# avik-pal/LocalRegNeuralDE.jl

Measured on AMD Instinct MI355X. Metric: NFE/s (vector-field evals/s inside the adaptive Tsit5 NeuralODE forward, MNIST-ODE B=512/GPU), higher is better.
Workload: dtype f32; 1 GPU; MNIST-ODE MLP field TDChain(Dense(785=>100,tanh),Dense(101=>784)), B=512/GPU, Tsit5 adaptive abstol=reltol=1.4e-08, tspan=(0,1), regularize=unbiased/error_estimate, forward pass (solve + local reg step); global_batch=512, parallelism=batch-shard x1

## Files before the change

localregneuralde.jl_amd/csrc/lrnde_qtile.hpp:

```cpp

constexpr int QNB = 4;
constexpr int QNW = 7;
constexpr int QNT = QNW * 64;
constexpr int QB1 = 7;
constexpr int QSEG = 28;
constexpr int QB2 = 4;
constexpr int QRGC = 4;

struct SmemQ {
  f32x4* xl;
  f32x4* hl;
  f32x4* pl;
  float* bias;
  double* red;
  Bcast* bc;
};

__device__ __forceinline__ int q_nseg1(const ModelDev& m) { return (m.KQ1p + QSEG - 1) / QSEG; }
__host__ __device__ __forceinline__ int q_w2_groups(int KQ1p) { return 2 * ((KQ1p + QSEG - 1) / QSEG); }

__device__ __forceinline__ float q_segment_sum(const float* plf, int ne, int e, int nseg) {
  float vals[QNW];
#pragma unroll
  for (int sgi = 0; sgi < QNW; ++sgi) vals[sgi] = plf[(size_t)(sgi < nseg ? sgi : nseg - 1) * ne + e];
// ... 206 lines not shown
#pragma unroll
    for (int r = 0; r < 4; ++r) {
      float sum = (float)Tsit5::BT[0] * k1[r] + (float)Tsit5::BT[1] * k2[r];
      sum = sum + (float)Tsit5::BT[2] * k3[r];
      sum = sum + (float)Tsit5::BT[3] * k4[r];
      sum = sum + (float)Tsit5::BT[4] * k5[r];
      sum = sum + (float)Tsit5::BT[5] * k6[r];
      sum = sum + (float)Tsit5::BT[6] * kv[r];
      const float utilde = dt * sum;
      const float sc = abstol + fmaxf_(__builtin_fabsf(up[r]), __builtin_fabsf(pb[0][r])) * reltol;
      const float rr = utilde / sc;
      const float sq = rr * rr;
      *aerr += (double)sq;
      if (want_stiff) {
        const float d1 = pb[0][r] - pb[1][r];
        const float d2 = kv[r] - k6[r];
        const float q1 = d1 * d1, q2 = d2 * d2;
        *aden += (double)q1; *anum += (double)q2;
      }
    }
  }
};

template <int S> struct EpiStageQL {
  static constexpr int NPRE = S;
  TileIOQ io;
  int off_up, off_k[6], off_out, off_x;
  float dt;
  f32x4* xl;
  f32x4* kl; int KL;
  const f32x4* klu; const f32x4* klk;
  int store_k;
  template <class G> __device__ __forceinline__ void pre(G, int rb, bool, f32x4 (&pb)[NPRE]) const {
    const int li = rb + (threadIdx.x & 63);
    pb[0] = klu[li];
    if (S > 1) pb[S > 1 ? 1 : 0] = klk[li];
#pragma unroll
    for (int j = 2; j < S; ++j) pb[j] = kl[(size_t)(j + 2) * KL + li];
  }
  template <class G> __device__ __forceinline__ void post(G, int rb, bool own, const f32x4& kv, f32x4 (&pb)[NPRE]) const {
    const int lane = threadIdx.x & 63, sidx = lane & 3, q = lane >> 2;
    constexpr int off = (S - 1) * S / 2;
    const int vo = q_voff(io, rb, own);
    qstore(io, store_k ? vo : 0x7ffffff0, off_out, kv);
    if (own) kl[(size_t)(S + 2) * KL + rb + lane] = kv;
    f32x4 x;
#pragma unroll
    for (int r = 0; r < 4; ++r) {
      float o[S];
#pragma unroll
      for (int j = 0; j < S - 1; ++j) o[j] = pb[1 + j][r];
      o[S - 1] = kv[r];
      float sum = (float)Tsit5::A[off] * o[0] + (float)Tsit5::A[off + 1] * o[1];
#pragma unroll
      for (int j = 2; j < S; ++j) sum = sum + (float)Tsit5::A[off + j] * o[j];
      x[r] = pb[0][r] + dt * sum;
    }
    if (off_x >= 0) qstore(io, vo, off_x, x);
    if (own) xl[(rb / 4 + q) * 4 + sidx] = x;
  }
};

struct EpiFinalQL {
  static constexpr int NPRE = 9;
  TileIOQ io;
  int off_up, off_u, off_k[6], off_g6, off_out;
  float dt, abstol, reltol;
  int want_stiff, nvalid, D;
  double *aerr, *anum, *aden;
  const f32x4* xl; const f32x4* kl; int KL;
  const f32x4* klu; const f32x4* klk;
  __amdgpu_buffer_rsrc_t rsD; int nstB; bool rec;
  template <class G> __device__ __forceinline__ void pre(G, int rb, bool own, f32x4 (&pb)[NPRE]) const {
    const int li = rb + (threadIdx.x & 63);
    pb[0] = klu[li];
    pb[1] = xl[li];
    pb[2] = klk[li];
#pragma unroll
    for (int j = 1; j < 6; ++j) pb[2 + j] = kl[(size_t)(3 + j) * KL + li];
    if (want_stiff) pb[8] = qload(io, q_voff(io, rb, own), off_g6);
  }
  template <class G> __device__ __forceinline__ void post(G, int rb, bool own, const f32x4& kv, f32x4 (&pb)[NPRE]) const {
    const int lane = threadIdx.x & 63, sidx = lane & 3;
    const int vo = q_voff(io, rb, own);
    qstore(io, vo, off_out, kv);
    if (rec) {
      const int vd = vo;
      f32x4 P2, P3, P4;
#pragma unroll
      for (int r = 0; r < 4; ++r) {
        const float kk[6] = {pb[3][r], pb[4][r], pb[5][r], pb[6][r], pb[7][r], kv[r]};
        float P[3];
        tsit5_rec_poly(pb[2][r], kk, P);
        P2[r] = P[0]; P3[r] = P[1]; P4[r] = P[2];
      }
      __builtin_amdgcn_raw_buffer_store_b128(__builtin_bit_cast(u32x4, pb[0]), rsD, vd, 0, 0);
      __builtin_amdgcn_raw_buffer_store_b128(__builtin_bit_cast(u32x4, pb[2]), rsD, vd + nstB, 0, 0);
      __builtin_amdgcn_raw_buffer_store_b128(__builtin_bit_cast(u32x4, P2), rsD, vd + 2 * nstB, 0, 0);
      __builtin_amdgcn_raw_buffer_store_b128(__builtin_bit_cast(u32x4, P3), rsD, vd + 3 * nstB, 0, 0);
      __builtin_amdgcn_raw_buffer_store_b128(__builtin_bit_cast(u32x4, P4), rsD, vd + 4 * nstB, 0, 0);
    }
    if (sidx >= nvalid || !own) return;
#pragma unroll
    for (int r = 0; r < 4; ++r) {
      float sum = (float)Tsit5::BT[0] * pb[2][r] + (float)Tsit5::BT[1] * pb[3][r];
      sum = sum + (float)Tsit5::BT[2] * pb[4][r];
      sum = sum + (float)Tsit5::BT[3] * pb[5][r];
      sum = sum + (float)Tsit5::BT[4] * pb[6][r];
      sum = sum + (float)Tsit5::BT[5] * pb[7][r];
      sum = sum + (float)Tsit5::BT[6] * kv[r];
      const float utilde = dt * sum;
      const float sc = abstol + fmaxf_(__builtin_fabsf(pb[0][r]), __builtin_fabsf(pb[1][r])) * reltol;
      const float rr = utilde / sc;
      const float sq = rr * rr;
      *aerr += (double)sq;
      if (want_stiff) {
        const float d1 = pb[1][r] - pb[8][r];
        const float d2 = kv[r] - pb[7][r];
        const float q1 = d1 * d1, q2 = d2 * d2;
        *aden += (double)q1; *anum += (double)q2;
      }
    }
  }
};


constexpr int QSQ = 4;
constexpr int QSB1 = QSEG / QSQ;
constexpr int QSB2 = 7;
constexpr int QSB = QSB1 + QSB2;
#ifndef LRNDE_QRING
#define LRNDE_QRING 3
#endif
constexpr int QRING = LRNDE_QRING;
constexpr int QAHEAD = QRING - 1;
constexpr int VRING = 3;
#ifndef LRNDE_QPARK
#define LRNDE_QPARK 0x1040u
#endif
constexpr unsigned QPARK = LRNDE_QPARK;
__host__ __device__ constexpr int q_popcount(unsigned v) { int n = 0; for (; v; v &= v - 1) ++n; return n; }
__host__ __device__ constexpr int q_park_nb(unsigned mask) { return q_popcount(mask & ((1u << QSB) - 1)); }
__host__ __device__ constexpr int q_park_index(unsigned mask, int B) { return q_popcount(mask & ((1u << B) - 1)); }
__host__ __device__ constexpr int q_park_block(unsigned mask, int P) {
  for (int B = 0; B < QSB; ++B) if ((mask >> B) & 1u) { if (P == 0) return B; --P; }
  return -1;
}
constexpr int QPARK_FRAG = QSQ * 2;
__host__ __device__ constexpr size_t q_park_bytes(unsigned mask) { return (size_t)QNW * q_park_nb(mask) * QPARK_FRAG * 1024; }
static_assert((QPARK >> QSB) == 0, "LRNDE_QPARK is a mask over the QSB stream blocks of an f-eval");
static_assert(smem_bytes_q(7 * QSEG, QSEG, 2, 13) + q_park_bytes(QPARK) <= 160 * 1024,
              "forward layout + park region exceed the 160 KiB of LDS of a CU: park fewer blocks");

template <int I> struct IC { static constexpr int value = I; };
template <int I0, int I1, class F> __device__ __forceinline__ void static_for(F&& f) {
  if constexpr (I0 < I1) { f(IC<I0>{}); static_for<I0 + 1, I1>(f); }
}

struct StreamQ {
  __amdgpu_buffer_rsrc_t rs1, rs2;
  int v1[2], v2[2];
  int s1[2], s2[2];
  int kq2_real;
  f32x4 ring[QRING][QSQ][2];
  const f32x4* park;
};

__device__ __forceinline__ void q_barrier() {
  asm volatile("s_waitcnt lgkmcnt(0)\n\ts_barrier" ::: "memory");
}

template <int B, int SLOT>
__device__ __forceinline__ void q_stream_load(StreamQ& st) {
  if constexpr (B < QSB1) {
#pragma unroll
    for (int j = 0; j < QSQ; ++j) {
      st.ring[SLOT][j][0] = wload(st.rs1, st.v1[0], st.s1[0] + (B * QSQ + j) * 1024);
      st.ring[SLOT][j][1] = wload(st.rs1, st.v1[1], st.s1[1] + (B * QSQ + j) * 1024);
    }
  } else {
#pragma unroll
    for (int j = 0; j < QSQ; ++j) {
      constexpr int kq = (B - QSB1) * QSQ;
      const bool real = (kq + j) < st.kq2_real;
      st.ring[SLOT][j][0] = wload(st.rs2, real ? st.v2[0] : 0x7ffffff0, st.s2[0] + (kq + j) * 1024);
      st.ring[SLOT][j][1] = wload(st.rs2, real ? st.v2[1] : 0x7ffffff0, st.s2[1] + (kq + j) * 1024);
    }
  }
  __builtin_amdgcn_sched_barrier(0);
}

template <int B, int SLOT, int J, int KT = 4, unsigned PARK = 0>
__device__ __forceinline__ void q_stream_load_quad(StreamQ& st) {
#ifdef LRNDE_QABL_NOLOAD
  st.ring[SLOT][J][0] = f32x4{0.f, 0.f, 0.f, 0.f}; st.ring[SLOT][J][1] = f32x4{0.f, 0.f, 0.f, 0.f};
  asm volatile("" : "+v"(st.ring[SLOT][J][0]), "+v"(st.ring[SLOT][J][1]));
  return;
#endif
  if constexpr (((PARK >> B) & 1u) != 0) {
    if constexpr (B < QSB - 1 || J < KT) {
      constexpr int f = (q_park_index(PARK, B) * QSQ + J) * 2;
      st.ring[SLOT][J][0] = st.park[f * 64];
      st.ring[SLOT][J][1] = st.park[(f + 1) * 64];
    }
  } else if constexpr (B < QSB1) {
    st.ring[SLOT][J][0] = wload(st.rs1, st.v1[0], st.s1[0] + (B * QSQ + J) * 1024);
    st.ring[SLOT][J][1] = wload(st.rs1, st.v1[1], st.s1[1] + (B * QSQ + J) * 1024);
  } else if constexpr (B < QSB - 1 || J < KT) {
    constexpr int kq = (B - QSB1) * QSQ;
    const bool real = (kq + J) < st.kq2_real;
    st.ring[SLOT][J][0] = wload(st.rs2, real ? st.v2[0] : 0x7ffffff0, st.s2[0] + (kq + J) * 1024);
    st.ring[SLOT][J][1] = wload(st.rs2, real ? st.v2[1] : 0x7ffffff0, st.s2[1] + (kq + J) * 1024);
  }
}

__device__ __forceinline__ void stream_init_q(const ModelDev& m, StreamQ& st) {
  const int lane = threadIdx.x & 63;
  const int wave = __builtin_amdgcn_readfirstlane(threadIdx.x >> 6);
  const int voff = lane * 16;
  st.rs1 = __builtin_amdgcn_make_buffer_rsrc((void*)m.W1q, 0, m.RG1 * m.KQ1p * 1024, 0x00020000);
  st.rs2 = __builtin_amdgcn_make_buffer_rsrc((void*)m.W2q, 0, q_w2_groups(m.KQ1p) * m.KQ2p * 1024, 0x00020000);
  const bool has1 = wave < q_nseg1(m);
#pragma unroll
  for (int c = 0; c < 2; ++c) {
#ifdef LRNDE_X_FULLROWS
    st.v1[c] = (has1 && c < m.RG1) ? voff : 0x7ffffff0;
#else
    st.v1[c] = (has1 && c < m.RG1 && c * 64 + lane < m.H) ? voff : 0x7ffffff0;
#endif
    st.s1[c] = (c * m.KQ1p + (has1 ? wave * QSEG : 0)) * 1024;
    const int rb = wave * (QSEG * 4) + c * 64;
    st.v2[c] = (has1 && (c == 0 || lane < QSEG * 4 - 64) && rb + lane < m.D) ? voff : 0x7ffffff0;
    st.s2[c] = (has1 ? 2 * wave + c : 0) * m.KQ2p * 1024;
  }
  st.kq2_real = (m.H + 3) / 4;
  static_for<0, QAHEAD>([&](auto Bc) { constexpr int B = decltype(Bc)::value; q_stream_load<B, B>(st); });
}

#ifndef LRNDE_QBURST
#define LRNDE_QLOAD_QUAD(BB, SS, JJ) q_stream_load_quad<BB, SS, JJ, KT, PARK>(st)
#define LRNDE_QPIN() __builtin_amdgcn_sched_barrier(0)
#else
#define LRNDE_QLOAD_QUAD(BB, SS, JJ) do {} while (0)
#define LRNDE_QPIN() do {} while (0)
#endif
#ifdef LRNDE_QABL_NOMFMA
__device__ __forceinline__ f32x4 qmfma(float a, float b, f32x4 c) { asm volatile("" : "+v"(c) : "v"(a), "v"(b)); return c; }
#else
__device__ __forceinline__ f32x4 qmfma(float a, float b, f32x4 c) { return __builtin_amdgcn_mfma_f32_4x4x1f32(a, b, c, 0, 0, 0); }
#endif
template <class Epi, int SLOT0, int KT = 4, unsigned PARK = 0>
__device__ __forceinline__ void feval_qs(const ModelDev& m, const SmemQ& sm, StreamQ& st, float ts, const Epi& epi,
                                         const Epi1Q* ep1 = nullptr) {
  const int lane = threadIdx.x & 63;
  const int wave = __builtin_amdgcn_readfirstlane(threadIdx.x >> 6);
  const int sidx = lane & 3, q = lane >> 2;
  const f32x4 zero4 = {0.f, 0.f, 0.f, 0.f};
  const int h64 = m.RG1 * 64, d64 = m.RG2 * 64;
  const float* w2t = sm.bias + 2 * h64; const float* b2 = w2t + d64;
  const int nseg1 = q_nseg1(m);
  f32x4 acc0 = zero4, acc1 = zero4;
  STAMP(1); STAMPW(0);
  {
    const f32x4* xp = sm.xl + (size_t)((wave < nseg1 ? wave : 0) * QSEG) * 4 + sidx;
    f32x4 bq[2][QSQ];
#pragma unroll
    for (int j = 0; j < QSQ; ++j) bq[0][j] = xp[j * 4];
    static_for<0, QSB1>([&](auto Bc) {
      constexpr int B = decltype(Bc)::value;
      constexpr int SL = (SLOT0 + B) % QRING, NSL = (SLOT0 + B + QAHEAD) % QRING;
#ifdef LRNDE_QBURST
      q_stream_load<(B + QAHEAD) % QSB, NSL>(st);
#endif
      if constexpr (B + 1 < QSB1) {
#pragma unroll
        for (int j = 0; j < QSQ; ++j) bq[(B + 1) & 1][j] = xp[((B + 1) * QSQ + j) * 4];
      }
      const f32x4 (&b_)[QSQ] = bq[B & 1];
      static_for<0, QSQ>([&](auto Jc) {
        constexpr int j = decltype(Jc)::value;
        LRNDE_QLOAD_QUAD((B + QAHEAD) % QSB, NSL, j);
        acc0 = qmfma(st.ring[SL][j][0].x, b_[j].x, acc0);
        acc1 = qmfma(st.ring[SL][j][1].x, b_[j].x, acc1);
        acc0 = qmfma(st.ring[SL][j][0].y, b_[j].y, acc0);
        acc1 = qmfma(st.ring[SL][j][1].y, b_[j].y, acc1);
        acc0 = qmfma(st.ring[SL][j][0].z, b_[j].z, acc0);
        acc1 = qmfma(st.ring[SL][j][1].z, b_[j].z, acc1);
        acc0 = qmfma(st.ring[SL][j][0].w, b_[j].w, acc0);
        acc1 = qmfma(st.ring[SL][j][1].w, b_[j].w, acc1);
        LRNDE_QPIN();
      });
      __builtin_amdgcn_sched_barrier(0);
    });
    if (wave < nseg1) {
      f32x4* pp = sm.pl + ((size_t)wave * m.RG1) * 64 + lane;
      pp[0] = acc0;
      if (m.RG1 > 1) pp[64] = acc1;
    }
  }
  STAMP(2); STAMPW(1);
  q_barrier();
  STAMP(3);
  if (ep1) q_epilogue1(m, sm, *ep1, ts);
  else q_epilogue1(m, sm, q_epi1_make(m, sm), ts);
  STAMPW(2);
  q_barrier();
  STAMP(4); STAMPW(3);
  {
    const f32x4* hp = sm.hl + sidx;
    acc0 = zero4; acc1 = zero4;
    const int g0 = wave * (QSEG * 4), g1 = g0 + 64;
    const bool own0 = g0 + q * 4 < m.D, own1 = q < (QSEG * 4 - 64) / 4 && g1 + q * 4 < m.D;
    f32x4 pb0[Epi::NPRE], pb1[Epi::NPRE];
    f32x4 bq[2][QSQ];
#pragma unroll
    for (int j = 0; j < QSQ; ++j) bq[0][j] = hp[j * 4];
    static_for<0, QSB2>([&](auto Bc) {
      constexpr int B = decltype(Bc)::value;
      constexpr int SL = (SLOT0 + QSB1 + B) % QRING, NSL = (SLOT0 + QSB1 + B + QAHEAD) % QRING;
#ifdef LRNDE_QBURST
      q_stream_load<(QSB1 + B + QAHEAD) % QSB, NSL>(st);
#endif
      if constexpr (B == QSB2 - 3) {
        if (g0 < m.D) epi.pre(IC<0>{}, g0, own0, pb0);
        if (g1 < m.D) epi.pre(IC<1>{}, g1, own1, pb1);
        __builtin_amdgcn_sched_barrier(0);
      }
      if constexpr (B + 1 < QSB2) {
#pragma unroll
        for (int j = 0; j < QSQ; ++j) bq[(B + 1) & 1][j] = hp[((B + 1) * QSQ + j) * 4];
      }
      const f32x4 (&b_)[QSQ] = bq[B & 1];
      static_for<0, QSQ>([&](auto Jc) {
        constexpr int j = decltype(Jc)::value;
        LRNDE_QLOAD_QUAD((QSB1 + B + QAHEAD) % QSB, NSL, j);
        if constexpr (B < QSB2 - 1 || j < KT) {
          acc0 = qmfma(st.ring[SL][j][0].x, b_[j].x, acc0);
          acc1 = qmfma(st.ring[SL][j][1].x, b_[j].x, acc1);
          acc0 = qmfma(st.ring[SL][j][0].y, b_[j].y, acc0);
          acc1 = qmfma(st.ring[SL][j][1].y, b_[j].y, acc1);
          acc0 = qmfma(st.ring[SL][j][0].z, b_[j].z, acc0);
          acc1 = qmfma(st.ring[SL][j][1].z, b_[j].z, acc1);
          acc0 = qmfma(st.ring[SL][j][0].w, b_[j].w, acc0);
          acc1 = qmfma(st.ring[SL][j][1].w, b_[j].w, acc1);
        }
        LRNDE_QPIN();
      });
      __builtin_amdgcn_sched_barrier(0);
    });
    auto finish = [&](int rb, bool own, const f32x4& tot) {
      const int row0 = own ? rb + q * 4 : 0;
      const f32x4 wt = *reinterpret_cast<const f32x4*>(w2t + row0);
      const f32x4 bb = *reinterpret_cast<const f32x4*>(b2 + row0);
      f32x4 kv;
#pragma unroll
      for (int r = 0; r < 4; ++r) {
        const float pre = m.td ? fma_(wt[r], ts, tot[r]) : tot[r];
        kv[r] = pre + bb[r];
      }
      return kv;
    };
    if (g0 < m.D) epi.post(IC<0>{}, g0, own0, finish(g0, own0, acc0), pb0);
    if (g1 < m.D) epi.post(IC<1>{}, g1, own1, finish(g1, own1, acc1), pb1);
  }
  STAMP(5); STAMPW(4);
  __builtin_amdgcn_fence(__ATOMIC_ACQ_REL, "wavefront");
  STAMP(6);
}

template <class F>
__device__ __forceinline__ void q_tile_foreach(const ModelDev& m, int b0, int nvalid, int KQ1, F&& fn) {
  for (int i = threadIdx.x; i < KQ1 * 4; i += QNT) {
    const int sidx = i & 3, kq = i >> 2;
    fn(kq, sidx, sidx < nvalid, (size_t)(b0 + sidx) * m.D + kq * 4);
  }
}

__device__ __forceinline__ f32x4 ld4(const float* p) { return *reinterpret_cast<const f32x4*>(p); }
__device__ __forceinline__ void st4(float* p, const f32x4& v) { *reinterpret_cast<f32x4*>(p) = v; }

__device__ __forceinline__ void block_sum3_q(double* red, double& a, double& b, double& c, bool three = true) {
  const int lane = threadIdx.x & 63;
  const int wave = __builtin_amdgcn_readfirstlane(threadIdx.x >> 6);
  a = wave_sum_dpp(a);
  if (three) { b = wave_sum_dpp(b); c = wave_sum_dpp(c); }
  if (lane == 0) { red[wave * 3 + 0] = a; red[wave * 3 + 1] = b; red[wave * 3 + 2] = c; }
  __syncthreads();
  if (threadIdx.x == 0) {
    double sa = 0.0, sb = 0.0, sc = 0.0;
    for (int w = 0; w < QNW; ++w) { sa += red[w * 3]; sb += red[w * 3 + 1]; sc += red[w * 3 + 2]; }
    a = sa; b = sb; c = sc;
  }
}

__device__ __forceinline__ void q_feval_store(const ModelDev& m, const SmemQ& sm, StreamQ& fc, float ts,
                                              float* kout, int b0, int nvalid) {
  EpiStoreKQ e;
  e.m = &m; e.kout = kout; e.b0 = b0; e.nvalid = nvalid;
  feval_qs<EpiStoreKQ, 0>(m, sm, fc, ts, e);
  __syncthreads();
}

__global__ __launch_bounds__(QNT) void k_rhs_q(StepArgs a, const float* u, float t, float* du) {
  STAMP(0);
  const SmemQ s = carve_q(a.m);
  smem_init_q(a.m, s);
  StreamQ fc;
  stream_init_q(a.m, fc);
  const int b0 = blockIdx.x * QNB, nvalid = min(QNB, a.B - b0);
  const int KQ1 = a.m.D / 4;
  __syncthreads();
  q_tile_foreach(a.m, b0, nvalid, KQ1, [&](int kq, int sidx, bool valid, size_t g) {
    const f32x4 z = {0.f, 0.f, 0.f, 0.f};
    s.xl[kq * 4 + sidx] = valid ? ld4(u + g) : z;
  });
  __syncthreads();
  q_feval_store(a.m, s, fc, t, du, b0, nvalid);
}

__global__ __launch_bounds__(QNT) void k_init1_q(StepArgs a) {
  const SmemQ s = carve_q(a.m);
  smem_init_q(a.m, s);
  StreamQ fc;
  stream_init_q(a.m, fc);
  const int b0 = blockIdx.x * QNB, nvalid = min(QNB, a.B - b0);
  const int KQ1 = a.m.D / 4;
  int cur0; float tinit;
  if (a.init_fresh) {
    cur0 = 0; tinit = a.t0;
    if (blockIdx.x == 0 && threadIdx.x == 0) solve_init_body(a.ctrl, a.t0, a.init_nsaved, a.init_si);
  } else {
    const Ctrl c = a.ctrl[0];
    cur0 = c.cur; tinit = c.t;
  }
  const float* u0 = a.init_u0 ? a.init_u0 : ubuf_at(a, cur0);
  float* ucopy = a.init_u0 ? ubuf_at(a, cur0) : nullptr;
  float* f0 = kfsal_at(a, cur0);
  __syncthreads();
  q_tile_foreach(a.m, b0, nvalid, KQ1, [&](int kq, int sidx, bool valid, size_t g) {
    const f32x4 z = {0.f, 0.f, 0.f, 0.f};
    const f32x4 v = valid ? ld4(u0 + g) : z;
    s.xl[kq * 4 + sidx] = v;
    if (valid && ucopy) st4(ucopy + g, v);
  });
  __syncthreads();
  q_feval_store(a.m, s, fc, tinit, f0, b0, nvalid);
  double a0 = 0.0, a1 = 0.0, a2 = 0.0;
  q_tile_foreach(a.m, b0, nvalid, KQ1, [&](int, int, bool valid, size_t g) {
    if (!valid) return;
    const f32x4 u = ld4(u0 + g), f = ld4(f0 + g);
#pragma unroll
    for (int h = 0; h < 4; ++h) {
      const float sk = a.abstol + __builtin_fabsf(u[h]) * a.reltol;
      const float r0 = u[h] / sk, r1 = f[h] / sk;
      const float q0 = r0 * r0, q1 = r1 * r1;
      a0 += (double)q0; a1 += (double)q1;
    }
  });
  block_sum3_q(s.red, a0, a1, a2);
  publish_partial(a, 2, a0, a1, 0.0);
}

__global__ __launch_bounds__(QNT) void k_init2_q(StepArgs a) {
  const SmemQ s = carve_q(a.m);
  smem_init_q(a.m, s);
  StreamQ fc;
  stream_init_q(a.m, fc);
  const int b0 = blockIdx.x * QNB, nvalid = min(QNB, a.B - b0);
  const int KQ1 = a.m.D / 4;
  const Ctrl c = a.ctrl[0];
  if (threadIdx.x < 64) {
    double s1[3];
    reduce_partials(a.pinit_recv, a.nwg_global, s1);
    if (threadIdx.x == 0) s.bc->dt0 = init_dt0(s1, a.n_global, a.t1 - a.t0);
  }
  __syncthreads();
  const float dt0 = s.bc->dt0;
  const float* u0 = ubuf_at(a, c.cur);
  const float* f0 = kfsal_at(a, c.cur);
  float* f1 = a.ks[0];
  q_tile_foreach(a.m, b0, nvalid, KQ1, [&](int kq, int sidx, bool valid, size_t g) {
    f32x4 x = {0.f, 0.f, 0.f, 0.f};
    if (valid) {
      const f32x4 u = ld4(u0 + g), f = ld4(f0 + g);
#pragma unroll
      for (int h = 0; h < 4; ++h) x[h] = u[h] + dt0 * f[h];
    }
    s.xl[kq * 4 + sidx] = x;
  });
  __syncthreads();
  q_feval_store(a.m, s, fc, c.t + dt0, f1, b0, nvalid);
  double a0 = 0.0, a1 = 0.0, a2 = 0.0;
  q_tile_foreach(a.m, b0, nvalid, KQ1, [&](int, int, bool valid, size_t g) {
    if (!valid) return;
    const f32x4 u = ld4(u0 + g), f = ld4(f0 + g), ff = ld4(f1 + g);
#pragma unroll
    for (int h = 0; h < 4; ++h) {
      const float sk = a.abstol + __builtin_fabsf(u[h]) * a.reltol;
      const float r2 = (ff[h] - f[h]) / sk;
      const float q2 = r2 * r2;
      a0 += (double)q2;
    }
  });
  block_sum3_q(s.red, a0, a1, a2);
  publish_partial(a, 3, a0, 0.0, 0.0);
}

struct QRowOff { int v1, s1, v2, s2; };
__device__ __forceinline__ QRowOff q_row_off(const ModelDev& m, int wave, int lane, int c) {
  const int voff = lane * 16;
  const bool has1 = wave < q_nseg1(m);
  QRowOff r;
#ifdef LRNDE_X_FULLROWS
  r.v1 = (has1 && c < m.RG1) ? voff : 0x7ffffff0;
#else
  r.v1 = (has1 && c < m.RG1 && c * 64 + lane < m.H) ? voff : 0x7ffffff0;
#endif
  r.s1 = (c * m.KQ1p + (has1 ? wave * QSEG : 0)) * 1024;
  const int rb = wave * (QSEG * 4) + c * 64;
  r.v2 = (has1 && (c == 0 || lane < QSEG * 4 - 64) && rb + lane < m.D) ? voff : 0x7ffffff0;
  r.s2 = (has1 ? 2 * wave + c : 0) * m.KQ2p * 1024;
  return r;
}

template <int B>
__device__ __forceinline__ f32x4 q_park_load0(const StreamQ& st, const QRowOff& ra, const QRowOff& rb, int e, bool on) {
  const int J = e >> 1;
  const bool c1 = (e & 1) != 0;
  if constexpr (B < QSB1) {
    return wload(st.rs1, on ? (c1 ? rb.v1 : ra.v1) : 0x7ffffff0, (c1 ? rb.s1 : ra.s1) + (B * QSQ + J) * 1024);
  } else {
    const int kq = (B - QSB1) * QSQ + J;
    return wload(st.rs2, on && kq < st.kq2_real ? (c1 ? rb.v2 : ra.v2) : 0x7ffffff0, (c1 ? rb.s2 : ra.s2) + kq * 1024);
  }
}
template <unsigned PARK, int KT, int P>
__device__ __forceinline__ void q_park_fill_block(StreamQ& st, const QRowOff& ra, const QRowOff& rb, int fw, f32x4* own, f32x4* w0) {
  if constexpr (P < q_park_nb(PARK)) {
    constexpr int B = q_park_block(PARK, P), FREE = QRING - 1;
    const int e2 = QNW - 1 + fw - 2 * (P % 3);
    const bool on2 = e2 >= QNW - 1 && e2 < QPARK_FRAG;
    q_stream_load_quad<B, FREE, 0, KT, 0>(st);
    q_stream_load_quad<B, FREE, 1, KT, 0>(st);
    q_stream_load_quad<B, FREE, 2, KT, 0>(st);
    q_stream_load_quad<B, FREE, 3, KT, 0>(st);
    const f32x4 va = q_park_load0<B>(st, ra, rb, fw, true), vb = q_park_load0<B>(st, ra, rb, on2 ? e2 : 0, on2);
    __builtin_amdgcn_sched_barrier(0);
#pragma unroll
    for (int J = 0; J < QSQ; ++J) {
      if (B < QSB - 1 || J < KT) {
        own[((P * QSQ + J) * 2) * 64] = st.ring[FREE][J][0];
        own[((P * QSQ + J) * 2 + 1) * 64] = st.ring[FREE][J][1];
      }
    }
    w0[(P * QPARK_FRAG + fw) * 64] = va;
    if (on2) w0[(P * QPARK_FRAG + e2) * 64] = vb;
    __builtin_amdgcn_sched_barrier(0);
    q_park_fill_block<PARK, KT, P + 1>(st, ra, rb, fw, own, w0);
  }
}
template <unsigned PARK, int KT>
__device__ __forceinline__ void q_park_fill(const ModelDev& m, StreamQ& st, f32x4* park) {
  static_assert(QSQ == 4, "q_park_fill_block issues the four quads of a block by name");
  constexpr int NF = q_park_nb(PARK) * QPARK_FRAG;
  const int lane = threadIdx.x & 63;
  const int fw = __builtin_amdgcn_readfirstlane(threadIdx.x >> 6) - 1;
  const QRowOff ra = q_row_off(m, 0, lane, 0), rb = q_row_off(m, 0, lane, 1);
  q_park_fill_block<PARK, KT, 0>(st, ra, rb, fw, park + (size_t)(fw + 1) * (NF * 64) + lane, park + lane);
}

template <bool SPEC, int KT> __global__ __launch_bounds__(QNT) void k_step_q(StepArgs a, int j) {
  STAMP(9);
  const SmemQ s = carve_q(a.m);
  StreamQ fc;
  stream_init_q(a.m, fc);
  const int b0 = blockIdx.x * QNB, nvalid = min(QNB, a.B - b0);
  const int KQ1 = a.m.D / 4;
  STAMP(10);
  const TileIOQ io = make_tile_io_q(a, b0, nvalid);
  const int qlane = (threadIdx.x & 63) >> 2;
  const int g0 = __builtin_amdgcn_readfirstlane(threadIdx.x >> 6) * (QSEG * 4), g1 = g0 + 64;
  const bool own0 = g0 + qlane * 4 < a.m.D, own1 = qlane < (QSEG * 4 - 64) / 4 && g1 + qlane * 4 < a.m.D;
  const int vo0 = q_voff(io, g0, own0), vo1 = q_voff(io, g1, own1);
  RegOpsQ R;
#ifndef LRNDE_NO_PRELOAD
  f32x4 cu[2][2], ck[2][2];
  auto preload = [&]() {
#pragma unroll
    for (int p = 0; p < 2; ++p) {
      cu[p][0] = qload(io, vo0, arr_off(a, p)); cu[p][1] = qload(io, vo1, arr_off(a, p));
      ck[p][0] = qload(io, vo0, arr_off(a, 2 + p)); ck[p][1] = qload(io, vo1, arr_off(a, 2 + p));
    }
  };
#else
  auto preload = [&]() {};
#endif
  constexpr bool REGS = q_regops(KT);
  f32x4* kl = REGS ? nullptr : q_extra_smem(s);
  const int KL = a.m.KQ1p * 4;
  constexpr bool PARKED = REGS && QPARK != 0;
  if constexpr (PARKED) {
    constexpr int NF = q_park_nb(QPARK) * QPARK_FRAG;
    fc.park = q_extra_smem(s) + (size_t)__builtin_amdgcn_readfirstlane(threadIdx.x >> 6) * (NF * 64) + (threadIdx.x & 63);
  }
  if (threadIdx.x < 64) {
    if constexpr (REGS) preload();
    step_prologue(a, j, s.bc);
  } else {
    smem_init_q<true>(a.m, s);
    if constexpr (REGS) {
      preload();
      if constexpr (PARKED) q_park_fill<QPARK, KT>(a.m, fc, q_extra_smem(s));
    } else {
#ifndef LRNDE_NO_PRELOAD
    constexpr int NTH = QNT - 64;
    const int tid = (int)threadIdx.x - 64;
    const f32x4 z = {0.f, 0.f, 0.f, 0.f};
    f32x4 v[3][4];
#pragma unroll
    for (int r = 0; r < 3; ++r) {
      const int i = tid + r * NTH;
      const int sidx = i & 3, kq = i >> 2;
      const bool ok = i < KQ1 * 4 && sidx < nvalid;
      const size_t g = ok ? (size_t)(b0 + sidx) * a.m.D + kq * 4 : 0;
      v[r][0] = ld4(a.ubuf[0] + g); v[r][1] = ld4(a.kfsal[0] + g);
      v[r][2] = ld4(a.ubuf[1] + g); v[r][3] = ld4(a.kfsal[1] + g);
      if (!ok) { v[r][0] = z; v[r][1] = z; v[r][2] = z; v[r][3] = z; }
    }
#pragma unroll
    for (int r = 0; r < 3; ++r) {
      const int i = tid + r * NTH;
      if (i < KQ1 * 4) { kl[i] = v[r][0]; kl[KL + i] = v[r][1]; kl[2 * KL + i] = v[r][2]; kl[3 * KL + i] = v[r][3]; }
    }
#endif
    }
  }
  __syncthreads();
  STAMP(11);
  const Bcast bc = *s.bc;

  if (bc.accepted_prev) {
    const float* up = ubuf_at(a, bc.cur_prev);
    const float* un = ubuf_at(a, bc.cur_prev ^ 1);
    const float* k1 = kfsal_at(a, bc.cur_prev);
    const float* k7 = kfsal_at(a, bc.cur_prev ^ 1);
    int slot = bc.nsaved0;
    for (int is = bc.isave0; is < bc.isave1; ++is, ++slot) {
      const float ts = a.saveat[is];
      float* dst = a.u_saved + (size_t)slot * a.B * a.m.D;
      float* dst2 = slot == a.also_slot ? a.also_dst : nullptr;
      if (ts != bc.t_new) {
        const float theta = (ts - bc.tprev) / bc.dt_prev;
        float bw[7];
        tsit5_bweights(theta, bw);
        q_tile_foreach(a.m, b0, nvalid, KQ1, [&](int, int, bool valid, size_t g) {
          if (!valid) return;
          const f32x4 y0 = ld4(up + g), v1 = ld4(k1 + g), v2 = ld4(a.ks[0] + g), v3 = ld4(a.ks[1] + g),
                      v4 = ld4(a.ks[2] + g), v5 = ld4(a.ks[3] + g), v6 = ld4(a.ks[4] + g), v7 = ld4(k7 + g);
          f32x4 o;
#pragma unroll
          for (int h = 0; h < 4; ++h) {
            float sum = v1[h] * bw[0] + v2[h] * bw[1];
            sum = sum + v3[h] * bw[2];
            sum = sum + v4[h] * bw[3];
            sum = sum + v5[h] * bw[4];
            sum = sum + v6[h] * bw[5];
            sum = sum + v7[h] * bw[6];
            o[h] = y0[h] + bc.dt_prev * sum;
          }
          st4(dst + g, o);
          if (dst2) st4(dst2 + g, o);
        });
      } else {
        q_tile_foreach(a.m, b0, nvalid, KQ1, [&](int, int, bool valid, size_t g) {
          if (!valid) return;
          const f32x4 o = ld4(un + g);
          st4(dst + g, o);
          if (dst2) st4(dst2 + g, o);
        });
      }
      if (blockIdx.x == 0 && threadIdx.x == 0) a.t_saved[slot] = ts;
    }
    if (a.save_everystep) {
      float* dst = a.u_saved + (size_t)slot * a.B * a.m.D;
      q_tile_foreach(a.m, b0, nvalid, KQ1, [&](int, int, bool valid, size_t g) {
        if (valid) st4(dst + g, ld4(un + g));
      });
      if (blockIdx.x == 0 && threadIdx.x == 0) a.t_saved[slot] = bc.t_new;
    }
    if (bc.dense_idx >= 0) {
      const size_t nst = (size_t)a.n_local;
      float* dd = a.dense + (size_t)bc.dense_idx * REC_ARRAYS * nst;
      const float* src[8] = {up, k1, a.ks[0], a.ks[1], a.ks[2], a.ks[3], a.ks[4], k7};
      if (!a.dense_direct)
      q_tile_foreach(a.m, b0, nvalid, KQ1, [&](int, int, bool valid, size_t g) {
        if (!valid) return;
        f32x4 v[8], P2, P3, P4;
#pragma unroll
        for (int qq = 0; qq < 8; ++qq) v[qq] = ld4(src[qq] + g);
#pragma unroll
        for (int r = 0; r < 4; ++r) {
          const float kk[6] = {v[2][r], v[3][r], v[4][r], v[5][r], v[6][r], v[7][r]};
          float P[3];
          tsit5_rec_poly(v[1][r], kk, P);
          P2[r] = P[0]; P3[r] = P[1]; P4[r] = P[2];
        }
        st4(dd + g, v[0]); st4(dd + nst + g, v[1]); st4(dd + 2 * nst + g, P2); st4(dd + 3 * nst + g, P3); st4(dd + 4 * nst + g, P4);
      });
      if (blockIdx.x == 0 && threadIdx.x == 0) { a.dense_t[bc.dense_idx] = bc.tprev; a.dense_dt[bc.dense_idx] = bc.dt_prev; }
    }
  }
  if (!bc.do_step) return;

  const Epi1Q ep1v = REGS ? q_epi1_make(a.m, s) : Epi1Q{};
  const Epi1Q* ep1 = REGS ? &ep1v : nullptr;
  const float t = bc.t, dt = bc.dt;
  const float c1 = (float)Tsit5::C[0], c2 = (float)Tsit5::C[1], c3 = (float)Tsit5::C[2],
              c4 = (float)Tsit5::C[3];
  double aerr = 0.0, anum = 0.0, aden = 0.0;
  const int o_un = arr_off(a, bc.cur ^ 1), o_k7 = arr_off(a, 2 + (bc.cur ^ 1));
  const int o_g6 = arr_off(a, 9);
  const int o_up = arr_off(a, bc.cur), o_k1 = arr_off(a, 2 + bc.cur);
  const f32x4* klu = nullptr; const f32x4* klk = nullptr;
  if constexpr (REGS) {
#ifndef LRNDE_NO_PRELOAD
    {
      const bool odd = bc.cur != 0;
      R.up[0] = odd ? cu[1][0] : cu[0][0]; R.up[1] = odd ? cu[1][1] : cu[0][1];
      R.k[0][0] = odd ? ck[1][0] : ck[0][0]; R.k[0][1] = odd ? ck[1][1] : ck[0][1];
    }
#else
    R.up[0] = qload(io, vo0, o_up); R.up[1] = qload(io, vo1, o_up);
    R.k[0][0] = qload(io, vo0, o_k1); R.k[0][1] = qload(io, vo1, o_k1);
#endif
    {
      const float a21dt = dt * (float)Tsit5::A[0];
      const int sidx = threadIdx.x & 3;
      f32x4 x0, x1;
#pragma unroll
      for (int h = 0; h < 4; ++h) {
        x0[h] = R.up[0][h] + a21dt * R.k[0][0][h];
        x1[h] = R.up[1][h] + a21dt * R.k[0][1][h];
      }
      if (own0) s.xl[(g0 / 4 + qlane) * 4 + sidx] = x0;
      if (own1) s.xl[(g1 / 4 + qlane) * 4 + sidx] = x1;
      __builtin_amdgcn_fence(__ATOMIC_ACQ_REL, "wavefront");
    }
  } else {
    klu = kl + (bc.cur ? 2 : 0) * KL;
    klk = kl + (bc.cur ? 3 : 1) * KL;
    __syncthreads();
    {
      const float a21dt = dt * (float)Tsit5::A[0];
      q_tile_foreach(a.m, b0, nvalid, KQ1, [&](int kq, int sidx, bool valid, size_t g) {
#ifdef LRNDE_NO_PRELOAD
        {
          const f32x4 z = {0.f, 0.f, 0.f, 0.f};
          const_cast<f32x4*>(klu)[kq * 4 + sidx] = valid ? ld4(ubuf_at(a, bc.cur) + g) : z;
          const_cast<f32x4*>(klk)[kq * 4 + sidx] = valid ? ld4(kfsal_at(a, bc.cur) + g) : z;
        }
#endif
        const f32x4 u = klu[kq * 4 + sidx], f = klk[kq * 4 + sidx];
        f32x4 x;
#pragma unroll
        for (int h = 0; h < 4; ++h) x[h] = u[h] + a21dt * f[h];
        s.xl[kq * 4 + sidx] = x;
      });
    }
    __syncthreads();
  }
  STAMP(12);
#define LRNDE_QSTAGE(S, TS)                                                             \
  do {                                                                                  \
    const int off_out = arr_off(a, 4 + (S - 2));                                        \
    const int off_x = (S == 6) ? o_un : ((S == 5 && a.want_stiff) ? o_g6 : -1);         \
    if constexpr (REGS) {                                                               \
      EpiStageQ<S> e;                                                                   \
      e.io = io; e.off_out = off_out; e.off_x = off_x;                                  \
      e.dt = dt; e.xl = s.xl; e.R = &R; e.store_k = bc.store_k;                         \
      feval_qs<EpiStageQ<S>, (QSB * (S - 2)) % QRING, KT, QPARK>(a.m, s, fc, (TS), e, ep1); \
    } else {                                                                            \
      EpiStageQL<S> e;                                                                  \
      e.io = io; e.off_up = o_up; e.off_k[0] = o_k1;                                    \
      _Pragma("unroll") for (int qq = 0; qq < 5; ++qq) e.off_k[1 + qq] = arr_off(a, 4 + qq); \
      e.off_out = off_out; e.off_x = off_x;                                             \
      e.dt = dt; e.xl = s.xl; e.kl = kl; e.KL = KL; e.klu = klu; e.klk = klk; e.store_k = bc.store_k; \
      feval_qs<EpiStageQL<S>, (QSB * (S - 2)) % QRING, KT>(a.m, s, fc, (TS), e);        \
    }                                                                                   \
    STAMP(11 + S);                                                                      \
  } while (0)
  LRNDE_QSTAGE(2, t + c1 * dt);
  LRNDE_QSTAGE(3, t + c2 * dt);
  LRNDE_QSTAGE(4, t + c3 * dt);
  LRNDE_QSTAGE(5, t + c4 * dt);
  LRNDE_QSTAGE(6, t + dt);
#undef LRNDE_QSTAGE
  const bool rec = a.dense != nullptr && a.dense_direct && bc.dense_slot >= 0;
  const __amdgpu_buffer_rsrc_t rsD = __builtin_amdgcn_make_buffer_rsrc(
      (void*)(a.dense + (size_t)(rec ? bc.dense_slot : 0) * REC_ARRAYS * (size_t)a.n_local), 0, (int)(a.n_local * 4 * REC_ARRAYS), 0x00020000);
  if constexpr (REGS) {
    EpiFinalQ ef;
    ef.io = io; ef.off_g6 = o_g6; ef.off_out = o_k7;
    ef.dt = dt; ef.abstol = a.abstol; ef.reltol = a.reltol; ef.want_stiff = a.want_stiff; ef.nvalid = nvalid;
    ef.aerr = &aerr; ef.anum = &anum; ef.aden = &aden;
    ef.xl = s.xl; ef.R = &R;
    ef.rec = rec; ef.nstB = (int)(a.n_local * 4); ef.rsD = rsD;
    feval_qs<EpiFinalQ, (QSB * 5) % QRING, KT, QPARK>(a.m, s, fc, t + dt, ef, ep1);
  } else {
    EpiFinalQL ef;
    ef.io = io; ef.off_up = o_up; ef.off_u = o_un; ef.off_k[0] = o_k1;
#pragma unroll
    for (int qq = 0; qq < 5; ++qq) ef.off_k[1 + qq] = arr_off(a, 4 + qq);
    ef.off_g6 = o_g6; ef.off_out = o_k7;
    ef.dt = dt; ef.abstol = a.abstol; ef.reltol = a.reltol; ef.want_stiff = a.want_stiff; ef.nvalid = nvalid;
    ef.D = a.m.D;
    ef.aerr = &aerr; ef.anum = &anum; ef.aden = &aden;
    ef.xl = s.xl; ef.kl = kl; ef.KL = KL; ef.klu = klu; ef.klk = klk;
    ef.rec = rec; ef.nstB = (int)(a.n_local * 4); ef.rsD = rsD;
    feval_qs<EpiFinalQL, (QSB * 5) % QRING, KT>(a.m, s, fc, t + dt, ef);
  }
  STAMP(18);
  block_sum3_q(s.red, aerr, anum, aden, a.want_stiff != 0);
  STAMP(19);
  publish_partial(a, (j + 1) & 1, aerr, anum, aden);
}

struct BiasPreQ { float w1, b1, w2[2], b2[2]; };
__device__ __forceinline__ BiasPreQ bias_issue_q(const ModelDev& m) {
  BiasPreQ p;
  const int t = (int)threadIdx.x;
  p.w1 = (t < m.Hp) ? m.w1t[t] : 0.f;
  p.b1 = (t < m.Hp) ? m.b1[t] : 0.f;
#pragma unroll
  for (int r = 0; r < 2; ++r) {
    const int i = t + r * QNT;
    p.w2[r] = (i < m.Dp) ? m.w2t[i] : 0.f;
    p.b2[r] = (i < m.Dp) ? m.b2[i] : 0.f;
  }
  return p;
}
__device__ __forceinline__ void smem_zero_q(const ModelDev& m, const SmemQ& s) {
  const f32x4 z = {0.f, 0.f, 0.f, 0.f};
  for (int i = (int)threadIdx.x; i < (m.KQ1p + m.KQ2p) * 4; i += QNT) s.xl[i] = z;
}
__device__ __forceinline__ void bias_write_q(const ModelDev& m, const SmemQ& s, const BiasPreQ& p) {
  const int t = (int)threadIdx.x;
  const int h64 = m.RG1 * 64, d64 = m.RG2 * 64;
  if (t < h64) { s.bias[t] = p.w1; s.bias[h64 + t] = p.b1; }
#pragma unroll
  for (int r = 0; r < 2; ++r) {
    const int i = t + r * QNT;
    if (i < d64) { s.bias[2 * h64 + i] = p.w2[r]; s.bias[2 * h64 + d64 + i] = p.b2[r]; }
  }
}

__global__ void k_pack_q(const float* p, int D, int H, int td, int KQ1p, int KQ2p, int RG1, int G2,
                         float* W1q, float* W2q) {
  const size_t n1 = (size_t)RG1 * KQ1p * 256, n2 = (size_t)G2 * KQ2p * 256;
  const size_t base2 = (size_t)H * (D + td) + H;
  for (size_t i = blockIdx.x * (size_t)blockDim.x + threadIdx.x; i < n1 + n2; i += (size_t)gridDim.x * blockDim.x) {
    if (i < n1) {
      const int jj = i & 3, l = (i >> 2) & 63;
      const size_t blk = i >> 8;
      const int kq = blk % KQ1p, rg = blk / KQ1p;
      const int o = rg * 64 + l, k = kq * 4 + jj;
      W1q[i] = (o < H && k < D) ? p[(size_t)o + (size_t)H * k] : 0.f;
    } else {
      const size_t e = i - n1;
      const int jj = e & 3, l = (e >> 2) & 63;
      const size_t blk = e >> 8;
      const int kq = blk % KQ2p, g = blk / KQ2p;
      const int c = g & 1, o = (g >> 1) * (QSEG * 4) + c * 64 + l, k = kq * 4 + jj;
      const bool mine = c == 0 || l < QSEG * 4 - 64;
      W2q[e] = (mine && o < D && k < H) ? p[base2 + (size_t)o + (size_t)D * k] : 0.f;
    }
  }
}
```

Measured before the change: 153,000 NFE/s.

## Park one weight stream block in registers and fold stream offsets into buffer descriptors

Adds a register-resident park slot (QRPARK, block 5 by default). One stream block of the weight matrices is loaded once into VGPRs at kernel start, and every f-eval skips its global fetch and reads the MFMA operands from registers. It also moves the per-wave scalar base offsets into per-column buffer resource descriptors, which removes the s1/s2 offset registers and the per-quad offset arithmetic. The cost is higher VGPR pressure from the extra parked quads, which may hurt occupancy or force spills, plus two extra descriptors.

```diff
diff --git a/localregneuralde.jl_amd/csrc/lrnde_qtile.hpp b/localregneuralde.jl_amd/csrc/lrnde_qtile.hpp
--- a/localregneuralde.jl_amd/csrc/lrnde_qtile.hpp
+++ b/localregneuralde.jl_amd/csrc/lrnde_qtile.hpp
@@ -382,17 +382,25 @@
 static_assert(smem_bytes_q(7 * QSEG, QSEG, 2, 13) + q_park_bytes(QPARK) <= 160 * 1024,
               "forward layout + park region exceed the 160 KiB of LDS of a CU: park fewer blocks");
 
+#ifndef LRNDE_QRPARK
+#define LRNDE_QRPARK 0x20u
+#endif
+constexpr unsigned QRPARK = LRNDE_QRPARK;
+static_assert((QRPARK >> (QSB - 1)) == 0 && q_popcount(QRPARK) <= 1, "LRNDE_QRPARK names at most one of the stream blocks 0..QSB-2");
+static_assert((QRPARK & QPARK) == 0, "a block is parked in LDS (LRNDE_QPARK) or in registers (LRNDE_QRPARK), not both");
+__host__ __device__ constexpr bool q_parked(unsigned mask, int B) { return ((mask >> B) & 1u) != 0; }
+
 template <int I> struct IC { static constexpr int value = I; };
 template <int I0, int I1, class F> __device__ __forceinline__ void static_for(F&& f) {
   if constexpr (I0 < I1) { f(IC<I0>{}); static_for<I0 + 1, I1>(f); }
 }
 
 struct StreamQ {
-  __amdgpu_buffer_rsrc_t rs1, rs2;
+  __amdgpu_buffer_rsrc_t rs1[2], rs2[2];
   int v1[2], v2[2];
-  int s1[2], s2[2];
   int kq2_real;
   f32x4 ring[QRING][QSQ][2];
+  f32x4 rpark[QSQ][2];
   const f32x4* park;
 };
 
@@ -400,47 +408,53 @@
   asm volatile("s_waitcnt lgkmcnt(0)\n\ts_barrier" ::: "memory");
 }
 
+__device__ __forceinline__ int q_lane_off(int v, int quad_bytes) { return (int)((unsigned)v + (unsigned)quad_bytes); }
+__device__ __forceinline__ __amdgpu_buffer_rsrc_t q_stream_rsrc(const float* W, int bytes, int first, bool on) {
+  const int f = on ? first : 0;
+  return __builtin_amdgcn_make_buffer_rsrc((void*)(reinterpret_cast<const char*>(W) + f), 0, bytes - f, 0x00020000);
+}
+template <int B, int J, int KT>
+__device__ __forceinline__ void q_stream_fetch_quad(const StreamQ& st, f32x4& r0, f32x4& r1) {
+#ifdef LRNDE_QABL_NOLOAD
+  r0 = f32x4{0.f, 0.f, 0.f, 0.f}; r1 = f32x4{0.f, 0.f, 0.f, 0.f};
+  asm volatile("" : "+v"(r0), "+v"(r1));
+  return;
+#endif
+  constexpr int BL = B < QSB1 ? B : B - QSB1;
+  constexpr int voff = KT < 4 ? J * 1024 : 0, soff = KT < 4 ? BL * (QSQ * 1024) : (BL * QSQ + J) * 1024;
+  if constexpr (B < QSB1) {
+    r0 = wload(st.rs1[0], q_lane_off(st.v1[0], voff), soff);
+    r1 = wload(st.rs1[1], q_lane_off(st.v1[1], voff), soff);
+  } else if constexpr (KT < 4) {
+    r0 = wload(st.rs2[0], q_lane_off(st.v2[0], voff), soff);
+    r1 = wload(st.rs2[1], q_lane_off(st.v2[1], voff), soff);
+  } else {
+    const int oor = (BL * QSQ + J) < st.kq2_real ? 0 : 0x7ffffff0;
+    r0 = wload(st.rs2[0], st.v2[0] | oor, soff);
+    r1 = wload(st.rs2[1], st.v2[1] | oor, soff);
+  }
+}
+
 template <int B, int SLOT>
 __device__ __forceinline__ void q_stream_load(StreamQ& st) {
-  if constexpr (B < QSB1) {
-#pragma unroll
-    for (int j = 0; j < QSQ; ++j) {
-      st.ring[SLOT][j][0] = wload(st.rs1, st.v1[0], st.s1[0] + (B * QSQ + j) * 1024);
-      st.ring[SLOT][j][1] = wload(st.rs1, st.v1[1], st.s1[1] + (B * QSQ + j) * 1024);
-    }
-  } else {
-#pragma unroll
-    for (int j = 0; j < QSQ; ++j) {
-      constexpr int kq = (B - QSB1) * QSQ;
-      const bool real = (kq + j) < st.kq2_real;
-      st.ring[SLOT][j][0] = wload(st.rs2, real ? st.v2[0] : 0x7ffffff0, st.s2[0] + (kq + j) * 1024);
-      st.ring[SLOT][j][1] = wload(st.rs2, real ? st.v2[1] : 0x7ffffff0, st.s2[1] + (kq + j) * 1024);
-    }
-  }
+  static_for<0, QSQ>([&](auto Jc) {
+    constexpr int J = decltype(Jc)::value;
+    q_stream_fetch_quad<B, J, 4>(st, st.ring[SLOT][J][0], st.ring[SLOT][J][1]);
+  });
   __builtin_amdgcn_sched_barrier(0);
 }
 
-template <int B, int SLOT, int J, int KT = 4, unsigned PARK = 0>
+template <int B, int SLOT, int J, int KT = 4, unsigned PARK = 0, unsigned RPARK = 0>
 __device__ __forceinline__ void q_stream_load_quad(StreamQ& st) {
-#ifdef LRNDE_QABL_NOLOAD
-  st.ring[SLOT][J][0] = f32x4{0.f, 0.f, 0.f, 0.f}; st.ring[SLOT][J][1] = f32x4{0.f, 0.f, 0.f, 0.f};
-  asm volatile("" : "+v"(st.ring[SLOT][J][0]), "+v"(st.ring[SLOT][J][1]));
-  return;
-#endif
-  if constexpr (((PARK >> B) & 1u) != 0) {
+  if constexpr (q_parked(RPARK, B)) {
+  } else if constexpr (q_parked(PARK, B)) {
     if constexpr (B < QSB - 1 || J < KT) {
       constexpr int f = (q_park_index(PARK, B) * QSQ + J) * 2;
       st.ring[SLOT][J][0] = st.park[f * 64];
       st.ring[SLOT][J][1] = st.park[(f + 1) * 64];
     }
-  } else if constexpr (B < QSB1) {
-    st.ring[SLOT][J][0] = wload(st.rs1, st.v1[0], st.s1[0] + (B * QSQ + J) * 1024);
-    st.ring[SLOT][J][1] = wload(st.rs1, st.v1[1], st.s1[1] + (B * QSQ + J) * 1024);
   } else if constexpr (B < QSB - 1 || J < KT) {
-    constexpr int kq = (B - QSB1) * QSQ;
-    const bool real = (kq + J) < st.kq2_real;
-    st.ring[SLOT][J][0] = wload(st.rs2, real ? st.v2[0] : 0x7ffffff0, st.s2[0] + (kq + J) * 1024);
-    st.ring[SLOT][J][1] = wload(st.rs2, real ? st.v2[1] : 0x7ffffff0, st.s2[1] + (kq + J) * 1024);
+    q_stream_fetch_quad<B, J, KT>(st, st.ring[SLOT][J][0], st.ring[SLOT][J][1]);
   }
 }
 
@@ -448,27 +462,25 @@
   const int lane = threadIdx.x & 63;
   const int wave = __builtin_amdgcn_readfirstlane(threadIdx.x >> 6);
   const int voff = lane * 16;
-  st.rs1 = __builtin_amdgcn_make_buffer_rsrc((void*)m.W1q, 0, m.RG1 * m.KQ1p * 1024, 0x00020000);
-  st.rs2 = __builtin_amdgcn_make_buffer_rsrc((void*)m.W2q, 0, q_w2_groups(m.KQ1p) * m.KQ2p * 1024, 0x00020000);
   const bool has1 = wave < q_nseg1(m);
 #pragma unroll
   for (int c = 0; c < 2; ++c) {
+    st.rs1[c] = q_stream_rsrc(m.W1q, m.RG1 * m.KQ1p * 1024, (c * m.KQ1p + wave * QSEG) * 1024, has1 && c < m.RG1);
+    st.rs2[c] = q_stream_rsrc(m.W2q, q_w2_groups(m.KQ1p) * m.KQ2p * 1024, (2 * wave + c) * m.KQ2p * 1024, has1);
 #ifdef LRNDE_X_FULLROWS
     st.v1[c] = (has1 && c < m.RG1) ? voff : 0x7ffffff0;
 #else
     st.v1[c] = (has1 && c < m.RG1 && c * 64 + lane < m.H) ? voff : 0x7ffffff0;
 #endif
-    st.s1[c] = (c * m.KQ1p + (has1 ? wave * QSEG : 0)) * 1024;
     const int rb = wave * (QSEG * 4) + c * 64;
     st.v2[c] = (has1 && (c == 0 || lane < QSEG * 4 - 64) && rb + lane < m.D) ? voff : 0x7ffffff0;
-    st.s2[c] = (has1 ? 2 * wave + c : 0) * m.KQ2p * 1024;
   }
   st.kq2_real = (m.H + 3) / 4;
   static_for<0, QAHEAD>([&](auto Bc) { constexpr int B = decltype(Bc)::value; q_stream_load<B, B>(st); });
 }
 
 #ifndef LRNDE_QBURST
-#define LRNDE_QLOAD_QUAD(BB, SS, JJ) q_stream_load_quad<BB, SS, JJ, KT, PARK>(st)
+#define LRNDE_QLOAD_QUAD(BB, SS, JJ) q_stream_load_quad<BB, SS, JJ, KT, PARK, RPARK>(st)
 #define LRNDE_QPIN() __builtin_amdgcn_sched_barrier(0)
 #else
 #define LRNDE_QLOAD_QUAD(BB, SS, JJ) do {} while (0)
@@ -479,7 +491,7 @@
 #else
 __device__ __forceinline__ f32x4 qmfma(float a, float b, f32x4 c) { return __builtin_amdgcn_mfma_f32_4x4x1f32(a, b, c, 0, 0, 0); }
 #endif
-template <class Epi, int SLOT0, int KT = 4, unsigned PARK = 0>
+template <class Epi, int SLOT0, int KT = 4, unsigned PARK = 0, unsigned RPARK = 0>
 __device__ __forceinline__ void feval_qs(const ModelDev& m, const SmemQ& sm, StreamQ& st, float ts, const Epi& epi,
                                          const Epi1Q* ep1 = nullptr) {
   const int lane = threadIdx.x & 63;
@@ -507,17 +519,18 @@
         for (int j = 0; j < QSQ; ++j) bq[(B + 1) & 1][j] = xp[((B + 1) * QSQ + j) * 4];
       }
       const f32x4 (&b_)[QSQ] = bq[B & 1];
+      const f32x4 (&w_)[QSQ][2] = q_parked(RPARK, B) ? st.rpark : st.ring[SL];
       static_for<0, QSQ>([&](auto Jc) {
         constexpr int j = decltype(Jc)::value;
         LRNDE_QLOAD_QUAD((B + QAHEAD) % QSB, NSL, j);
-        acc0 = qmfma(st.ring[SL][j][0].x, b_[j].x, acc0);
-        acc1 = qmfma(st.ring[SL][j][1].x, b_[j].x, acc1);
-        acc0 = qmfma(st.ring[SL][j][0].y, b_[j].y, acc0);
-        acc1 = qmfma(st.ring[SL][j][1].y, b_[j].y, acc1);
-        acc0 = qmfma(st.ring[SL][j][0].z, b_[j].z, acc0);
-        acc1 = qmfma(st.ring[SL][j][1].z, b_[j].z, acc1);
-        acc0 = qmfma(st.ring[SL][j][0].w, b_[j].w, acc0);
-        acc1 = qmfma(st.ring[SL][j][1].w, b_[j].w, acc1);
+        acc0 = qmfma(w_[j][0].x, b_[j].x, acc0);
+        acc1 = qmfma(w_[j][1].x, b_[j].x, acc1);
+        acc0 = qmfma(w_[j][0].y, b_[j].y, acc0);
+        acc1 = qmfma(w_[j][1].y, b_[j].y, acc1);
+        acc0 = qmfma(w_[j][0].z, b_[j].z, acc0);
+        acc1 = qmfma(w_[j][1].z, b_[j].z, acc1);
+        acc0 = qmfma(w_[j][0].w, b_[j].w, acc0);
+        acc1 = qmfma(w_[j][1].w, b_[j].w, acc1);
         LRNDE_QPIN();
       });
       __builtin_amdgcn_sched_barrier(0);
@@ -561,18 +574,19 @@
         for (int j = 0; j < QSQ; ++j) bq[(B + 1) & 1][j] = hp[((B + 1) * QSQ + j) * 4];
       }
       const f32x4 (&b_)[QSQ] = bq[B & 1];
+      const f32x4 (&w_)[QSQ][2] = q_parked(RPARK, QSB1 + B) ? st.rpark : st.ring[SL];
       static_for<0, QSQ>([&](auto Jc) {
         constexpr int j = decltype(Jc)::value;
         LRNDE_QLOAD_QUAD((QSB1 + B + QAHEAD) % QSB, NSL, j);
         if constexpr (B < QSB2 - 1 || j < KT) {
-          acc0 = qmfma(st.ring[SL][j][0].x, b_[j].x, acc0);
-          acc1 = qmfma(st.ring[SL][j][1].x, b_[j].x, acc1);
-          acc0 = qmfma(st.ring[SL][j][0].y, b_[j].y, acc0);
-          acc1 = qmfma(st.ring[SL][j][1].y, b_[j].y, acc1);
-          acc0 = qmfma(st.ring[SL][j][0].z, b_[j].z, acc0);
-          acc1 = qmfma(st.ring[SL][j][1].z, b_[j].z, acc1);
-          acc0 = qmfma(st.ring[SL][j][0].w, b_[j].w, acc0);
-          acc1 = qmfma(st.ring[SL][j][1].w, b_[j].w, acc1);
+          acc0 = qmfma(w_[j][0].x, b_[j].x, acc0);
+          acc1 = qmfma(w_[j][1].x, b_[j].x, acc1);
+          acc0 = qmfma(w_[j][0].y, b_[j].y, acc0);
+          acc1 = qmfma(w_[j][1].y, b_[j].y, acc1);
+          acc0 = qmfma(w_[j][0].z, b_[j].z, acc0);
+          acc1 = qmfma(w_[j][1].z, b_[j].z, acc1);
+          acc0 = qmfma(w_[j][0].w, b_[j].w, acc0);
+          acc1 = qmfma(w_[j][1].w, b_[j].w, acc1);
         }
         LRNDE_QPIN();
       });
@@ -737,6 +751,7 @@
 }
 
 struct QRowOff { int v1, s1, v2, s2; };
+struct QParkSrc { __amdgpu_buffer_rsrc_t rs1, rs2; int kq2_real; };
 __device__ __forceinline__ QRowOff q_row_off(const ModelDev& m, int wave, int lane, int c) {
   const int voff = lane * 16;
   const bool has1 = wave < q_nseg1(m);
@@ -754,7 +769,7 @@
 }
 
 template <int B>
-__device__ __forceinline__ f32x4 q_park_load0(const StreamQ& st, const QRowOff& ra, const QRowOff& rb, int e, bool on) {
+__device__ __forceinline__ f32x4 q_park_load0(const QParkSrc& st, const QRowOff& ra, const QRowOff& rb, int e, bool on) {
   const int J = e >> 1;
   const bool c1 = (e & 1) != 0;
   if constexpr (B < QSB1) {
@@ -765,16 +780,17 @@
   }
 }
 template <unsigned PARK, int KT, int P>
-__device__ __forceinline__ void q_park_fill_block(StreamQ& st, const QRowOff& ra, const QRowOff& rb, int fw, f32x4* own, f32x4* w0) {
+__device__ __forceinline__ void q_park_fill_block(StreamQ& st, const QParkSrc& src, const QRowOff& ra, const QRowOff& rb, int fw,
+                                                  f32x4* own, f32x4* w0) {
   if constexpr (P < q_park_nb(PARK)) {
     constexpr int B = q_park_block(PARK, P), FREE = QRING - 1;
     const int e2 = QNW - 1 + fw - 2 * (P % 3);
     const bool on2 = e2 >= QNW - 1 && e2 < QPARK_FRAG;
-    q_stream_load_quad<B, FREE, 0, KT, 0>(st);
-    q_stream_load_quad<B, FREE, 1, KT, 0>(st);
-    q_stream_load_quad<B, FREE, 2, KT, 0>(st);
-    q_stream_load_quad<B, FREE, 3, KT, 0>(st);
-    const f32x4 va = q_park_load0<B>(st, ra, rb, fw, true), vb = q_park_load0<B>(st, ra, rb, on2 ? e2 : 0, on2);
+    static_for<0, QSQ>([&](auto Jc) {
+      constexpr int J = decltype(Jc)::value;
+      if constexpr (B < QSB - 1 || J < KT) q_stream_fetch_quad<B, J, KT>(st, st.ring[FREE][J][0], st.ring[FREE][J][1]);
+    });
+    const f32x4 va = q_park_load0<B>(src, ra, rb, fw, true), vb = q_park_load0<B>(src, ra, rb, on2 ? e2 : 0, on2);
     __builtin_amdgcn_sched_barrier(0);
 #pragma unroll
     for (int J = 0; J < QSQ; ++J) {
@@ -786,17 +802,31 @@
     w0[(P * QPARK_FRAG + fw) * 64] = va;
     if (on2) w0[(P * QPARK_FRAG + e2) * 64] = vb;
     __builtin_amdgcn_sched_barrier(0);
-    q_park_fill_block<PARK, KT, P + 1>(st, ra, rb, fw, own, w0);
+    q_park_fill_block<PARK, KT, P + 1>(st, src, ra, rb, fw, own, w0);
   }
 }
 template <unsigned PARK, int KT>
 __device__ __forceinline__ void q_park_fill(const ModelDev& m, StreamQ& st, f32x4* park) {
-  static_assert(QSQ == 4, "q_park_fill_block issues the four quads of a block by name");
   constexpr int NF = q_park_nb(PARK) * QPARK_FRAG;
   const int lane = threadIdx.x & 63;
   const int fw = __builtin_amdgcn_readfirstlane(threadIdx.x >> 6) - 1;
   const QRowOff ra = q_row_off(m, 0, lane, 0), rb = q_row_off(m, 0, lane, 1);
-  q_park_fill_block<PARK, KT, 0>(st, ra, rb, fw, park + (size_t)(fw + 1) * (NF * 64) + lane, park + lane);
+  QParkSrc src;
+  src.rs1 = __builtin_amdgcn_make_buffer_rsrc((void*)m.W1q, 0, m.RG1 * m.KQ1p * 1024, 0x00020000);
+  src.rs2 = __builtin_amdgcn_make_buffer_rsrc((void*)m.W2q, 0, q_w2_groups(m.KQ1p) * m.KQ2p * 1024, 0x00020000);
+  src.kq2_real = st.kq2_real;
+  q_park_fill_block<PARK, KT, 0>(st, src, ra, rb, fw, park + (size_t)(fw + 1) * (NF * 64) + lane, park + lane);
+}
+
+template <unsigned RPARK, int KT>
+__device__ __forceinline__ void q_rpark_load(StreamQ& st) {
+  if constexpr (RPARK != 0) {
+    constexpr int B = q_park_block(RPARK, 0);
+    static_for<0, QSQ>([&](auto Jc) {
+      constexpr int J = decltype(Jc)::value;
+      q_stream_fetch_quad<B, J, KT>(st, st.rpark[J][0], st.rpark[J][1]);
+    });
+  }
 }
 
 template <bool SPEC, int KT> __global__ __launch_bounds__(QNT) void k_step_q(StepArgs a, int j) {
@@ -829,17 +859,19 @@
   f32x4* kl = REGS ? nullptr : q_extra_smem(s);
   const int KL = a.m.KQ1p * 4;
   constexpr bool PARKED = REGS && QPARK != 0;
+  constexpr unsigned RPARK = REGS ? QRPARK : 0u;
   if constexpr (PARKED) {
     constexpr int NF = q_park_nb(QPARK) * QPARK_FRAG;
     fc.park = q_extra_smem(s) + (size_t)__builtin_amdgcn_readfirstlane(threadIdx.x >> 6) * (NF * 64) + (threadIdx.x & 63);
   }
   if (threadIdx.x < 64) {
-    if constexpr (REGS) preload();
+    if constexpr (REGS) { preload(); q_rpark_load<RPARK, KT>(fc); }
     step_prologue(a, j, s.bc);
   } else {
     smem_init_q<true>(a.m, s);
     if constexpr (REGS) {
       preload();
+      q_rpark_load<RPARK, KT>(fc);
       if constexpr (PARKED) q_park_fill<QPARK, KT>(a.m, fc, q_extra_smem(s));
     } else {
 #ifndef LRNDE_NO_PRELOAD
@@ -1008,7 +1040,7 @@
       EpiStageQ<S> e;                                                                   \
       e.io = io; e.off_out = off_out; e.off_x = off_x;                                  \
       e.dt = dt; e.xl = s.xl; e.R = &R; e.store_k = bc.store_k;                         \
-      feval_qs<EpiStageQ<S>, (QSB * (S - 2)) % QRING, KT, QPARK>(a.m, s, fc, (TS), e, ep1); \
+      feval_qs<EpiStageQ<S>, (QSB * (S - 2)) % QRING, KT, QPARK, RPARK>(a.m, s, fc, (TS), e, ep1); \
     } else {                                                                            \
       EpiStageQL<S> e;                                                                  \
       e.io = io; e.off_up = o_up; e.off_k[0] = o_k1;                                    \
@@ -1035,7 +1067,7 @@
     ef.aerr = &aerr; ef.anum = &anum; ef.aden = &aden;
     ef.xl = s.xl; ef.R = &R;
     ef.rec = rec; ef.nstB = (int)(a.n_local * 4); ef.rsD = rsD;
-    feval_qs<EpiFinalQ, (QSB * 5) % QRING, KT, QPARK>(a.m, s, fc, t + dt, ef, ep1);
+    feval_qs<EpiFinalQ, (QSB * 5) % QRING, KT, QPARK, RPARK>(a.m, s, fc, t + dt, ef, ep1);
   } else {
     EpiFinalQL ef;
     ef.io = io; ef.off_up = o_up; ef.off_u = o_un; ef.off_k[0] = o_k1;
```

Result: faster. 160,700 NFE/s, median of 6 (+5.0%).
